# MohamedAbou-Taleb/Iterative-Linear-Quadratic-Regulator

Hardware: AMD Instinct MI355X
Metric: iLQR iterations/sec (batch=4096, T=200, n=4 m=1); backward-pass HBM GB/s (higher is better)
Workload: dtype f32; 1 GPU; c3: under-actuated double pendulum swing-up (run_iLQR_UA_MPC.py params), n=4 m=1 N=200 rk4, batch 4096 trajectories per GPU, 10 parallel line-search alphas per pass covering the 10 reference trials, fixed iterations; batch_per_gpu=4096, horizon=200, n_alpha=10, n_trials=10

## Files before the change

### iterative-linear-quadratic-regulator_amd/csrc/backward_fused16.hpp

```cpp
#pragma once

namespace ilqr {

template <typename T, int TPW, bool PK> struct FusedCfg;
template <> struct FusedCfg<float, 16, false> { static constexpr int P = 8, RU = 8; };
#ifndef ILQR_PK_RU
#define ILQR_PK_RU 5
#endif
#ifndef ILQR_PK_PAD
#define ILQR_PK_PAD 0
#endif
template <> struct FusedCfg<float, 16, true> { static constexpr int P = 4, RU = ILQR_PK_RU; };
template <> struct FusedCfg<double, 16, false> { static constexpr int P = 4, RU = 4; };
template <> struct FusedCfg<float, 4, false> { static constexpr int P = 3, RU = 4; };
template <> struct FusedCfg<double, 4, false> { static constexpr int P = 3, RU = 3; };

template <int NU> constexpr int fused_tl() { return NU == 2 ? 68 : 52; }
template <bool PK, int NU> constexpr int fused_unit_scalars() { return (PK ? 128 : 64) * fused_tl<NU>() + (PK ? 64 * ILQR_PK_PAD : 0); }
template <typename T, int TPW, bool PK, int NU> constexpr int fused_ru() { return (PK && NU == 2 && FusedCfg<T, TPW, PK>::RU > 4) ? 4 : FusedCfg<T, TPW, PK>::RU; }
template <typename T, int TPW, bool PK, int NU = 1> constexpr int fused_lds_bytes() {
    return fused_ru<T, TPW, PK, NU>() * fused_unit_scalars<PK, NU>() * (int)sizeof(T) + (fused_ru<T, TPW, PK, NU>() + 4 + 32 + 4) * 4;
}
static_assert(fused_lds_bytes<float, 16, true, 1>() <= 160 * 1024 && fused_lds_bytes<float, 16, true, 2>() <= 160 * 1024 &&
              fused_lds_bytes<float, 16, false, 2>() <= 160 * 1024 && fused_lds_bytes<double, 16, false, 2>() <= 160 * 1024, "LDS ring exceeds a CU");
template <typename T, int TPW, bool PK> constexpr int fused_threads() { return 64 * (TPW / 4 + FusedCfg<T, TPW, PK>::P); }

template <typename T, int NU> struct FusedStep;
template <> struct FusedStep<float, 1> {
    using Tile = TileQ;
    static ILQR_DEV void load(Tile& t, const float* tp, int i, int j, int l16) {
        const float4 s = *reinterpret_cast<const float4*>(tp + 4 * j);
        const float4 v = *reinterpret_cast<const float4*>(tp + 32 + 4 * j);
        t.skj[0] = s.x; t.skj[1] = s.y; t.skj[2] = s.z; t.skj[3] = s.w;
        t.vj[0] = v.x; t.vj[1] = v.y; t.vj[2] = v.z; t.vj[3] = v.w;
        t.a = tp[l16];
        t.lxx = tp[16 + l16];
        t.c = tp[32 + l16];
    }
    static ILQR_DEV void step(const Tile& c, const LaneConst<float>& lc, int i, int j, float& V, float& vx, float& out, bool& pd) {
        RawTileQ none;
        const i32x4 srd = {0, 0, 0, 0};
        const TileOffsets off = {0, 0, 0};
        float Kj, kff;
        tile16_step_f32<false>(c, lc, V, vx, Kj, kff, pd, none, srd, off, 0);
        out = (i == 0) ? Kj : kff;
    }
    static ILQR_DEV void step_box(const Tile& c, const LaneConst<float>& lc, int i, int j, float u, float lo, float hi,
                                  float& V, float& vx, float& out, bool& pd) {
        RawTileQ none;
        const i32x4 srd = {0, 0, 0, 0};
        const TileOffsets off = {0, 0, 0};
        float Kj, kff;
        tile16_step_f32<false, true>(c, lc, V, vx, Kj, kff, pd, none, srd, off, 0, u, lo, hi);
        out = (i == 0) ? Kj : kff;
    }
};
template <> struct FusedStep<double, 1> {
    using Tile = Tile16<double>;
    static ILQR_DEV void load(Tile& t, const double* tp, int i, int j, int l16) { tile16_load_lds(t, tp, i, j, l16); }
    static ILQR_DEV void step(const Tile& c, const LaneConst<double>& lc, int i, int j, double& V, double& vx, double& out, bool& pd) {
        double Kj, kff;
        tile16_step<double, false>(c, lc, 0.0, V, vx, Kj, kff, pd);
        out = (i == 0) ? Kj : kff;
    }
    static ILQR_DEV void step_box(const Tile& c, const LaneConst<double>& lc, int i, int j, double u, double lo, double hi,
                                  double& V, double& vx, double& out, bool& pd) {
        double Kj, kff;
        tile16_step<double, false, true>(c, lc, 0.0, V, vx, Kj, kff, pd, u, lo, hi);
        out = (i == 0) ? Kj : kff;
    }
};
template <> struct FusedStep<float, 2> {
    using Tile = TileQ2;
    static ILQR_DEV void load(Tile& t, const float* tp, int i, int j, int l16) { tileq2_load_lds(t, tp, i, j, l16); }
    static ILQR_DEV void step(const Tile& c, const LaneConst<float>& lc, int i, int j, float& V, float& vx, float& out, bool& pd) {
        const GainSel sel = GainSel::of(i, j);
        tile16m2_step_f32(c, lc, sel, V, vx, out, pd);
    }
};
template <typename T> struct FusedStep<T, 2> {
    using Tile = Tile16M2<T>;
    using V4 = typename Vec4<T>::type;
    static ILQR_DEV void load(Tile& t, const T* tp, int i, int j, int l16) {
        const V4 si = *reinterpret_cast<const V4*>(tp + 4 * i);
        const V4 sj = *reinterpret_cast<const V4*>(tp + 4 * j);
        const V4 g0 = *reinterpret_cast<const V4*>(tp + 32 + 8 * j);
        const V4 g1 = *reinterpret_cast<const V4*>(tp + 36 + 8 * j);
        t.ski[0] = si.x; t.ski[1] = si.y; t.ski[2] = si.z; t.ski[3] = si.w;
        t.skj[0] = sj.x; t.skj[1] = sj.y; t.skj[2] = sj.z; t.skj[3] = sj.w;
        t.gj[0] = g0.x; t.gj[1] = g0.y; t.gj[2] = g0.z; t.gj[3] = g0.w;
        t.gj[4] = g1.x; t.gj[5] = g1.y; t.gj[6] = g1.z; t.gj[7] = g1.w;
        const T* gi = tp + 32 + 8 * i;
        t.gi[0] = gi[0]; t.gi[1] = gi[1]; t.gi[3] = gi[3]; t.gi[4] = gi[4];
        t.lxx = tp[16 + l16];
    }
    static ILQR_DEV void step(const Tile& c, const LaneConst<T>& lc, int i, int j, T& V, T& vx, T& out, bool& pd) {
        T K0, K1, k0, k1;
        tile16m2_step<T, false>(c, lc.m0, lc.m1, T(0), V, vx, K0, K1, k0, k1, pd);
        out = (i == 0) ? K0 : ((i == 1) ? K1 : ((j == 0) ? k0 : k1));
    }
};

ILQR_DEV void compiler_fence() { asm volatile("" ::: "memory"); }
ILQR_DEV int lds_peek(const int* p) { return __hip_atomic_load(p, __ATOMIC_RELAXED, __HIP_MEMORY_SCOPE_WORKGROUP); }
ILQR_DEV void lds_poke(int* p, int v) { __hip_atomic_store(p, v, __ATOMIC_RELAXED, __HIP_MEMORY_SCOPE_WORKGROUP); }

template <typename T, typename Dyn, int INTEG, int TPW, bool PK, bool BOX, bool HET> struct FusedRoles {
    static constexpr int NX = Dyn::NX, NU = Dyn::NU;
    static_assert(!BOX || (NU == 1 && fused_tl<1>() > kTile16), "control limits: n_u = 1, u_t in the tile's padding");
    static_assert((NU == 1 && NX >= 2 && NX <= 4) || (NX == 4 && NU == 2), "the fused sweep serves the DPP tiles: n_u = 1, or (4, 2)");
    static_assert(TPW == 16 || TPW == 4, "16 or 4 trajectories per workgroup");
    static_assert(!PK || (sizeof(T) == 4 && TPW == 16 && INTEG != ILQR_INT_BACKWARD_EULER), "pair producers: fp32, 16-trajectory workgroups, explicit integrators");
    using Cfg = FusedCfg<T, TPW, PK>;
    static constexpr int P = Cfg::P, RU = fused_ru<T, TPW, PK, NU>(), TL = fused_tl<NU>();
    static constexpr int NV = (NU == 2 ? kTile16M2 : kTile16) / 4;
    static constexpr int NSW = TPW / 4;
    static constexpr int UT = PK ? 128 : 64;
    static constexpr int US = UT / TPW;
    static constexpr int UNIT = fused_unit_scalars<PK, NU>();
    static constexpr int PS = 2 * TL + ILQR_PK_PAD;
    static constexpr int R = gain_record(NX, NU);
    using PL = ParamLayout<Dyn::NSYS, NX, NU>;
    using V4 = typename Vec4<T>::type;
    static ILQR_DEV constexpr int tile_off(int r, int tl) { return PK ? ((r / 2) * TPW + tl) * PS + (r % 2) * TL : (r * TPW + tl) * TL; }
    static ILQR_DEV constexpr int step_off(int r) { return PK ? (r / 2) * TPW * PS + (r % 2) * TL : r * TPW * TL; }

    struct Lds {
        T* ring;
        int* ready;
        int* done;
        int* s_slot;
        int* s_stat;
    };
    static ILQR_DEV Lds carve(unsigned char* base) {
        Lds L;
        L.ring = reinterpret_cast<T*>(base);
        L.ready = reinterpret_cast<int*>(base + (size_t)RU * UNIT * sizeof(T));
        L.done = L.ready + RU;
        L.s_slot = L.done + 4;
        L.s_stat = L.s_slot + 16;
        return L;
    }

    static ILQR_DEV void head(const KArgs<T>& a, const Lds& L, int b0, int lane, bool do_select, bool count) {
        bool still = false;
        if (lane < 16) {
            const int b = b0 + lane;
            int slot = 0, st = -1;
            if (lane < TPW && b < a.B) {
                if (do_select) {
                    still = select_candidates(a, b, true, slot, st);
                } else {
                    st = a.status[b];
                    slot = a.cur_slot[b];
                }
                a.cur_slot[b] = traj_active(st) ? 0 : slot;
            }
            L.s_slot[lane] = slot;
            L.s_stat[lane] = st;
        } else if (lane < 16 + RU + 4) {
            L.ready[lane - 16] = 0;
        }
        if (do_select && count) {
            const unsigned long long m = __ballot(still);
            if (lane == 0 && m) atomicAdd(&a.counters[a.counter_idx], (int)__popcll(m));
            if (blockIdx.x == 0 && lane == 0) a.counters[(a.counter_idx + 1) % kCounterRing] = 0;
        }
    }
    static ILQR_DEV bool any_active(const Lds& L) {
        bool any = false;
#pragma unroll
        for (int q = 0; q < 16; ++q) any = any || traj_active(L.s_stat[q]);
        return any;
    }

    static ILQR_DEV void sweep(const KArgs<T>& a, const Lds& L, int b0, int wave, int lane, ClockProbe& cp) {
        const size_t B = a.B;
        const int N = a.N;
        const int tid = threadIdx.x;
        (void)tid;
        __builtin_amdgcn_s_setprio(2);
        const int l16 = lane & 15, i = l16 >> 2, j = l16 & 3;
        const int tl = 4 * wave + (lane >> 4);
        const int gidx = b0 + tl;
        const bool valid = gidx < a.B;
        const int b = valid ? gidx : a.B - 1;
        const int st = L.s_stat[tl];
        const bool act = valid && traj_active(st);
        const int slot = act ? L.s_slot[tl] : 0;
        T ph[HET ? PL::TOTAL : 1];
        if constexpr (HET) {
#pragma unroll
            for (int q = 0; q < PL::TOTAL; ++q) ph[q] = a.params[q];
            load_row<PL::Q>(ph, a.rows, B, b);
        }
        const T* __restrict__ pp = HET ? ph : a.params;
        T xN[NX];
        vec_load<T, NX>(a.X + vec_at(B, N + 1, NX, slot, N, b), xN);
        if (act && slot != 0 && l16 == 0) vec_store<T, NX>(a.X + vec_at(B, N + 1, NX, 0, N, b), xN);
        T V = T(0), vx = T(0);
        {
            T g[NX], H[NX][NX];
            Cost<T, Dyn>::l_f_x(pp, xN, g);
            Cost<T, Dyn>::l_f_xx(pp, xN, H);
#pragma unroll
            for (int ii = 0; ii < NX; ++ii) {
                if (j == ii) vx = g[ii];
#pragma unroll
                for (int jj = 0; jj < NX; ++jj)
                    if (i == ii && j == jj) V = H[ii][jj];
            }
        }
        const unsigned gain_bytes = (unsigned)((size_t)N * B * R * sizeof(T));
        const __amdgpu_buffer_rsrc_t rgain = make_rsrc(a.gains, gain_bytes);
        const int rstride = (int)(B * R * sizeof(T));
        constexpr bool DROP = sizeof(T) == 4 || ILQR_DROP_ALL;
        const bool storer = act && (NU == 1 ? ((i == 0 && j < NX) || l16 == 4) : (i < 2 || (i == 2 && j < 2)));
        const int rec_slot = NU == 1 ? (i == 0 ? j : NX) : (i < 2 ? 4 * i + j : 8 + j);
        const int rec_off = (storer || !DROP) ? (int)((b * R + rec_slot) * sizeof(T)) : 0x7ffffff0;
        LaneConst<T> lc;
        lc.m0 = T(j == 0);
        lc.m1 = T(j == 1);
        lc.tr_byte = 4 * ((lane & 48) | (j << 2) | i);
        bool all_pd = true;
        using FS = FusedStep<T, NU>;
        T blo = T(0), bhi = T(0);
        if constexpr (BOX) box_bounds<1>(a.lim, a.B, b, &blo, &bhi);
        typename FS::Tile tq[2];
        T uq[2] = {T(0), T(0)};
        auto load = [&](int q, const T* tp) {
            FS::load(tq[q], tp, i, j, l16);
            if constexpr (BOX) uq[q] = tp[kTile16];
        };
        int goff = (N - 1) * rstride;
        auto unit_base = [&](int k) -> const T* { return L.ring + (size_t)(k % RU) * UNIT + tile_off(0, tl); };
        constexpr auto step_off = [](int r) { return PK ? (r / 2) * TPW * PS + (r % 2) * TL : r * TPW * TL; };
        auto one_step = [&](int q) {
            T out;
            bool pd;
            if constexpr (BOX) FS::step_box(tq[q], lc, i, j, uq[q], blo, bhi, V, vx, out, pd);
            else FS::step(tq[q], lc, i, j, V, vx, out, pd);
            all_pd = all_pd && pd;
            if (DROP || storer) buf_store1(rgain, rec_off, uniform(goff), out);
            goff -= rstride;
        };
#ifdef ILQR_FUSED_STAMPS
        const long long st_t0 = __builtin_readcyclecounter();
        long long st_spin = 0;
#endif
        while (lds_peek(&L.ready[0]) < 1) __builtin_amdgcn_s_sleep(1);
        compiler_fence();
#ifdef ILQR_FUSED_STAMPS
        const long long st_first = __builtin_readcyclecounter();
#endif
        load(0, unit_base(0));
        const int n_full = N / US, rem = N % US;
        for (int k = 0; k < n_full; ++k) {
            const T* ub = unit_base(k);
            const bool more = (k + 1) * US < N;
            int flag = 0;
#pragma unroll
            for (int r = 0; r < US; ++r) {
                if (r == US - 2 && more) flag = lds_peek(&L.ready[(k + 1) % RU]);
                if (r < US - 1) {
                    load((r + 1) & 1, ub + step_off(r + 1));
                } else if (more) {
#ifdef ILQR_FUSED_STAMPS
                    const long long w0 = __builtin_readcyclecounter();
#endif
                    while (flag < k + 2) {
                        __builtin_amdgcn_s_sleep(1);
                        flag = lds_peek(&L.ready[(k + 1) % RU]);
                    }
                    compiler_fence();
#ifdef ILQR_FUSED_STAMPS
                    st_spin += __builtin_readcyclecounter() - w0;
#endif
                    load(0, unit_base(k + 1));
                }
                one_step(r & 1);
            }
            compiler_fence();
            if (lane == 0) lds_poke(&L.done[wave], k + 1);
        }
        if (rem) {
            const T* ub = unit_base(n_full);
#pragma unroll
            for (int r = 0; r < US - 1; ++r) {
                if (r < rem) {
                    if (r + 1 < rem) load((r + 1) & 1, ub + step_off(r + 1));
                    one_step(r & 1);
                }
            }
        }
#ifdef ILQR_FUSED_STAMPS
        if (a.probe && blockIdx.x == 7 && tid == 0) {
            a.probe[5] = st_first - st_t0;
            a.probe[6] = st_spin;
            a.probe[7] = __builtin_readcyclecounter() - st_first;
        }
#endif
        cp.stop(a.probe, 0);
        if (act && l16 == 0 && !all_pd) a.status[b] = st | ILQR_TRAJ_FLAG_NON_PD;
    }

    static ILQR_DEV void produce(const KArgs<T>& a_, const Lds& L, int b0, int pw, int lane) {
        struct { int B; T dt; T* X; T* U; const T* params; const T* rows; } a = {a_.B, a_.dt, a_.X, a_.U, a_.params, a_.rows};
        const size_t B = a.B;
        const int N = a_.N;
        const int n_units = (N + US - 1) / US;
        if constexpr (PK) {
        using T2 = pair_f32;
        using Dyn2 = typename Dyn::template rebind<T2>;
        const int tl = lane % TPW, r2 = lane / TPW;
        const int gidx = b0 + tl;
        const bool valid = gidx < a.B;
        const int b = valid ? gidx : a.B - 1;
        const bool actb = valid && traj_active(L.s_stat[tl]);
        const int slot = actb ? L.s_slot[tl] : 0;
        const bool move = actb && slot != 0;
        T pl[PL::TOTAL];
#pragma unroll
        for (int q = 0; q < PL::TOTAL; ++q) pl[q] = a.params[q];
        if constexpr (HET) load_row<PL::Q>(pl, a.rows, B, b);
        const SplatParams p{pl};
        const T2 dt2 = a.dt;
        for (int k = pw; k < n_units; k += P) {
            const int ta = N - 1 - k * US - 2 * r2, tb = ta - 1;
            const bool ina = ta >= 0, inb = tb >= 0;
            const int tta = ina ? ta : 0, ttb = inb ? tb : 0;
            T xa[NX], ua[NU], xb[NX], ub[NU];
            vec_load<T, NX>(a.X + vec_at(B, N + 1, NX, slot, tta, b), xa);
            vec_load<T, NU>(a.U + vec_at(B, N, NU, slot, tta, b), ua);
            vec_load<T, NX>(a.X + vec_at(B, N + 1, NX, slot, ttb, b), xb);
            vec_load<T, NU>(a.U + vec_at(B, N, NU, slot, ttb, b), ub);
            if (move && ina) {
                vec_store<T, NX>(a.X + vec_at(B, N + 1, NX, 0, tta, b), xa);
                vec_store<T, NU>(a.U + vec_at(B, N, NU, 0, tta, b), ua);
            }
            if (move && inb) {
                vec_store<T, NX>(a.X + vec_at(B, N + 1, NX, 0, ttb, b), xb);
                vec_store<T, NU>(a.U + vec_at(B, N, NU, 0, ttb, b), ub);
            }
            T2 x[NX], u[NU], xn[NX], fx[NX][NX], fu[NX][NU];
#pragma unroll
            for (int q = 0; q < NX; ++q) { x[q].x = xa[q]; x[q].y = xb[q]; }
#pragma unroll
            for (int q = 0; q < NU; ++q) { u[q].x = ua[q]; u[q].y = ub[q]; }
            Stepper<T2, Dyn2>::step_jac(INTEG, p, dt2, x, u, xn, fx, fu);
            T2 gxn[NX], gu1[NU], lxxn[NX][NX], luxn[NU][NX], luu[NU][NU];
            Cost<T2, Dyn2>::grad(p, dt2, x, u, gxn, gu1);
            Cost<T2, Dyn2>::hess(p, dt2, x, u, lxxn, luxn, luu);
            V4 tile_a[NV], tile_b[NV];
            tile16_fill<T, NX, NU>([](T2 v) { return v.x; }, fx, fu, gxn, gu1, lxxn, luxn, luu, tile_a);
            tile16_fill<T, NX, NU>([](T2 v) { return v.y; }, fx, fu, gxn, gu1, lxxn, luxn, luu, tile_b);
            if (k >= RU) {
                const int need = k - RU + 1;
                auto slowest = [&]() {
                    int m = lds_peek(&L.done[0]);
#pragma unroll
                    for (int q = 1; q < NSW; ++q) m = min(m, lds_peek(&L.done[q]));
                    return m;
                };
                while (slowest() < need) __builtin_amdgcn_s_sleep(2);
            }
            compiler_fence();
            V4* dst = reinterpret_cast<V4*>(L.ring + (size_t)(k % RU) * UNIT + tile_off(2 * r2, tl));
            if (ina) {
#pragma unroll
                for (int q = 0; q < NV; ++q) dst[q] = tile_a[q];
            }
            if (inb) {
#pragma unroll
                for (int q = 0; q < NV; ++q) dst[TL / 4 + q] = tile_b[q];
            }
            if constexpr (BOX) {
                T* dt_ = reinterpret_cast<T*>(dst);
                if (ina) dt_[kTile16] = ua[0];
                if (inb) dt_[TL + kTile16] = ub[0];
            }
            compiler_fence();
            if (lane == 0) lds_poke(&L.ready[k % RU], k + 1);
        }
        } else {
        const int tl = lane % TPW, r = lane / TPW;
        const int gidx = b0 + tl;
        const bool valid = gidx < a.B;
        const int b = valid ? gidx : a.B - 1;
        const bool actb = valid && traj_active(L.s_stat[tl]);
        const int slot = actb ? L.s_slot[tl] : 0;
        const bool move = actb && slot != 0;
        T p[PL::TOTAL];
#pragma unroll
        for (int q = 0; q < PL::TOTAL; ++q) p[q] = a.params[q];
        if constexpr (HET) load_row<PL::Q>(p, a.rows, B, b);
        for (int k = pw; k < n_units; k += P) {
            const int t = N - 1 - k * US - r;
            const bool inr = t >= 0;
            const int tt = inr ? t : 0;
            T x[NX], u[NU];
            vec_load<T, NX>(a.X + vec_at(B, N + 1, NX, slot, tt, b), x);
            vec_load<T, NU>(a.U + vec_at(B, N, NU, slot, tt, b), u);
            if (move && inr) {
                vec_store<T, NX>(a.X + vec_at(B, N + 1, NX, 0, tt, b), x);
                vec_store<T, NU>(a.U + vec_at(B, N, NU, 0, tt, b), u);
            }
            T xn[NX], fx[NX][NX], fu[NX][NU];
            Stepper<T, Dyn>::step_jac(INTEG, p, a.dt, x, u, xn, fx, fu);
            V4 tile[NV];
            tile16_pack<T, Dyn>(p, a.dt, x, u, fx, fu, tile);
            if (k >= RU) {
                const int need = k - RU + 1;
                auto slowest = [&]() {
                    int m = lds_peek(&L.done[0]);
#pragma unroll
                    for (int q = 1; q < NSW; ++q) m = min(m, lds_peek(&L.done[q]));
                    return m;
                };
                while (slowest() < need) __builtin_amdgcn_s_sleep(2);
            }
            compiler_fence();
            if (inr) {
                constexpr int NQ = NV * (int)sizeof(V4) / 16;
                vec_u4 w[NQ];
                __builtin_memcpy(w, tile, sizeof(V4) * NV);
                vec_u4* dst = reinterpret_cast<vec_u4*>(L.ring + (size_t)(k % RU) * UNIT + tile_off(r, tl));
#pragma unroll
                for (int q = 0; q < NQ; ++q) dst[q] = w[q];
                if constexpr (BOX) reinterpret_cast<T*>(dst)[kTile16] = u[0];
            }
            compiler_fence();
            if (lane == 0) lds_poke(&L.ready[k % RU], k + 1);
        }
        }
    }
};

template <typename T, typename Dyn, int INTEG, int TPW, bool PK, bool BOX = false>
struct FusedWG : FusedRoles<T, Dyn, INTEG, TPW, PK, BOX, false> {};
template <typename T, typename Dyn, int INTEG, int TPW, bool PK, bool BOX = false>
struct FusedWGHet : FusedRoles<T, Dyn, INTEG, TPW, PK, BOX, true> {};

template <typename T, typename Dyn, int INTEG, int TPW, bool PK, bool BOX = false, bool HET = false>
__global__ void __launch_bounds__((fused_threads<T, TPW, PK>())) backward_fused16_kernel(KArgs<T> a) {
    using W = std::conditional_t<HET, FusedWGHet<T, Dyn, INTEG, TPW, PK, BOX>, FusedWG<T, Dyn, INTEG, TPW, PK, BOX>>;
    extern __shared__ __attribute__((aligned(16))) unsigned char fused_lds[];
    const typename W::Lds L = W::carve(fused_lds);
    const int tid = threadIdx.x, wave = tid >> 6, lane = tid & 63;
    const int b0 = blockIdx.x * TPW;
    ClockProbe cp;
    cp.start();
    if (wave == 0) W::head(a, L, b0, lane, a.fuse_select != 0, true);
    __syncthreads();
    if (!W::any_active(L)) return;
    if (wave < W::NSW) W::sweep(a, L, b0, wave, lane, cp);
    else W::produce(a, L, b0, wave - W::NSW, lane);
}

}
```

### iterative-linear-quadratic-regulator_amd/csrc/kernels.hpp

```cpp
#pragma once
#include "dynamics.hpp"

namespace ilqr {

#ifndef ILQR_NT_TILE_STORE
#define ILQR_NT_TILE_STORE 0
#endif
#ifndef ILQR_NT_TILE_LOAD
#define ILQR_NT_TILE_LOAD 0
#endif
#ifndef ILQR_DROP_ALL
#define ILQR_DROP_ALL 0
#endif
constexpr int kMaxAlpha = 16;
constexpr int kCounterRing = 64;
constexpr int kBoxMaxU = 2;
constexpr int kALMaxX = 4;

template <typename T> struct Limits {
    T u_lo[kBoxMaxU], u_hi[kBoxMaxU];
    T x_lo[kALMaxX], x_hi[kALMaxX];
    int al_mask;
    const T* u_lo_rows;
    const T* u_hi_rows;
// ... 35 lines not shown
#pragma unroll
    for (int j = 0; j < NU; ++j) {
        lo[j] = rl ? rl[(size_t)j * B + b] : a.u_lo[j];
        hi[j] = rl ? rh[(size_t)j * B + b] : a.u_hi[j];
    }
}

template <int NH, typename T> ILQR_DEV void load_row(T* p, const T* __restrict__ rows, size_t B, int b) {
#pragma unroll
    for (int q = 0; q < NH; ++q) p[q] = rows[(size_t)q * B + b];
}

constexpr int gain_record(int nx, int nu) { return ((nu * nx + nu) + 3) / 4 * 4; }

ILQR_DEV bool traj_active(int status) { return (status & 0xff) == ILQR_TRAJ_ACTIVE; }

template <typename T> ILQR_DEV T clamp_keep_nan(T v, T lo, T hi) { return v < lo ? lo : (v > hi ? hi : v); }

ILQR_DEV size_t vec_at(size_t B, int Tn, int C, int slot, int t, size_t b) {
    return ((((size_t)slot * Tn + t) * B) + b) * C;
}
typedef unsigned int vec_u4 __attribute__((ext_vector_type(4)));
typedef unsigned int vec_u2 __attribute__((ext_vector_type(2)));
constexpr int vec_piece(int bytes) { return bytes % 16 == 0 ? 16 : bytes % 8 == 0 ? 8 : 4; }
constexpr int vec_pieces(int bytes) { return bytes / vec_piece(bytes); }
template <typename T, int C> ILQR_DEV void vec_load(const T* __restrict__ p, T* o) {
    constexpr int BYTES = C * (int)sizeof(T), PB = vec_piece(BYTES), NP = BYTES / PB;
    if constexpr (PB == 16) {
        vec_u4 v[NP];
#pragma unroll
        for (int k = 0; k < NP; ++k) v[k] = reinterpret_cast<const vec_u4*>(p)[k];
        __builtin_memcpy(o, v, BYTES);
    } else if constexpr (PB == 8) {
        vec_u2 v[NP];
#pragma unroll
        for (int k = 0; k < NP; ++k) v[k] = reinterpret_cast<const vec_u2*>(p)[k];
        __builtin_memcpy(o, v, BYTES);
    } else {
#pragma unroll
        for (int i = 0; i < C; ++i) o[i] = p[i];
    }
}
template <typename T, int C> ILQR_DEV void vec_store(T* __restrict__ p, const T* v) {
    constexpr int BYTES = C * (int)sizeof(T), PB = vec_piece(BYTES), NP = BYTES / PB;
    if constexpr (PB == 16) {
        vec_u4 w[NP];
        __builtin_memcpy(w, v, BYTES);
#pragma unroll
        for (int k = 0; k < NP; ++k) reinterpret_cast<vec_u4*>(p)[k] = w[k];
    } else if constexpr (PB == 8) {
        vec_u2 w[NP];
        __builtin_memcpy(w, v, BYTES);
#pragma unroll
        for (int k = 0; k < NP; ++k) reinterpret_cast<vec_u2*>(p)[k] = w[k];
    } else {
#pragma unroll
        for (int i = 0; i < C; ++i) p[i] = v[i];
    }
}

struct ClockProbe {
    long long c0, r0;
    ILQR_DEV void start() { c0 = __builtin_readcyclecounter(); r0 = wall_clock64(); }
    ILQR_DEV void stop(long long* probe, int slot) const {
        if (probe && threadIdx.x == 0) {
            const long long c1 = __builtin_readcyclecounter(), r1 = wall_clock64();
            const size_t wg = (size_t)blockIdx.y * gridDim.x + blockIdx.x;
            if (wg == 0) { probe[2 * slot] = c1 - c0; probe[2 * slot + 1] = r1 - r0; }
            if (wg < 65536) {
                long long* q = probe + 8 + ((size_t)slot * 65536 + wg) * 4;
                q[0] = r0; q[1] = r1; q[2] = c1 - c0;
                q[3] = (long long)__builtin_amdgcn_s_getreg((4 ) | (0 << 6) | (31 << 11)) |
                       ((long long)__builtin_amdgcn_s_getreg((20 ) | (0 << 6) | (3 << 11)) << 32);
            }
        }
    }
};

}
#include "backward_tile16.hpp"
#include "backward_tile16m2.hpp"
namespace ilqr {

template <typename TS, int NX, int NU, typename T, typename Pick>
ILQR_DEV void tile16_fill(Pick pick, const T (*fx)[NX], const T (*fu)[NU], const T* gxn, const T* gu1, const T (*lxxn)[NX],
                          const T (*luxn)[NX], const T (*luu)[NU], typename Vec4<TS>::type* tile) {
    static_assert((NX >= 2 && NX <= 4 && NU == 1) || (NX == 4 && NU == 2), "tile packing: n_x <= 4 with n_u = 1, or (4, 2)");
    auto F = [&](int i, int j) -> TS { return (i < NX && j < NX) ? pick(fx[i < NX ? i : 0][j < NX ? j : 0]) : TS(0); };
    auto L = [&](int i, int j) -> TS { return (i < NX && j < NX) ? pick(lxxn[i < NX ? i : 0][j < NX ? j : 0]) : TS(0); };
#pragma unroll
    for (int c = 0; c < 4; ++c) {
        tile[c].x = F((c + 0) & 3, c); tile[c].y = F((c + 1) & 3, c);
        tile[c].z = F((c + 2) & 3, c); tile[c].w = F((c + 3) & 3, c);
    }
#pragma unroll
    for (int i = 0; i < 4; ++i) {
        tile[4 + i].x = L(i, 0); tile[4 + i].y = L(i, 1);
        tile[4 + i].z = L(i, 2); tile[4 + i].w = L(i, 3);
    }
    if constexpr (NU == 1) {
#pragma unroll
        for (int j = 0; j < 4; ++j) {
            const int jj = j < NX ? j : 0;
            tile[8 + j].x = j < NX ? pick(fu[jj][0]) : TS(0);
            tile[8 + j].y = j < NX ? pick(gxn[jj]) : TS(0);
            tile[8 + j].z = j < NX ? pick(luxn[0][jj]) : TS(0);
            tile[8 + j].w = (j == 0) ? pick(gu1[0]) : ((j == 1) ? pick(luu[0][0]) : TS(0));
        }
    } else {
#pragma unroll
        for (int j = 0; j < 4; ++j) {
            tile[8 + 2 * j].x = pick(fu[j][0]); tile[8 + 2 * j].y = pick(fu[j][NU - 1]);
            tile[8 + 2 * j].z = pick(gxn[j]); tile[8 + 2 * j].w = pick(luxn[0][j]);
            tile[9 + 2 * j].x = pick(luxn[NU - 1][j]);
            tile[9 + 2 * j].y = (j == 0) ? pick(gu1[0]) : ((j == 1) ? TS(0.5) * (pick(luu[0][NU - 1]) + pick(luu[NU - 1][0])) : TS(0));
            tile[9 + 2 * j].z = (j == 0) ? pick(gu1[NU - 1]) : ((j == 1) ? pick(luu[NU - 1][NU - 1]) : TS(0));
            tile[9 + 2 * j].w = (j == 0) ? pick(luu[0][0]) : TS(0);
        }
    }
}

template <typename T, typename Dyn, typename P>
ILQR_DEV void tile16_pack(P p, T dt, const T* x, const T* u, const T (*fx)[Dyn::NX],
                          const T (*fu)[Dyn::NU], typename Vec4<T>::type* tile) {
    constexpr int NX = Dyn::NX, NU = Dyn::NU;
    T gxn[NX], gu1[NU], lxxn[NX][NX], luxn[NU][NX], luu[NU][NU];
    Cost<T, Dyn>::grad(p, dt, x, u, gxn, gu1);
    Cost<T, Dyn>::hess(p, dt, x, u, lxxn, luxn, luu);
    tile16_fill<T, NX, NU>([](T v) { return v; }, fx, fu, gxn, gu1, lxxn, luxn, luu, tile);
}

template <typename T, int NX> struct ALBounds {
    T lo[NX], hi[NX];
    int mask;
    ILQR_DEV ALBounds(const Limits<T>& a, size_t B, int b) : mask(a.al_mask) {
        const T* __restrict__ rl = a.x_lo_rows;
        const T* __restrict__ rh = a.x_hi_rows;
#pragma unroll
        for (int i = 0; i < NX; ++i) {
            lo[i] = rl ? rl[(size_t)i * B + b] : a.x_lo[i];
            hi[i] = rl ? rh[(size_t)i * B + b] : a.x_hi[i];
        }
    }
};
template <typename T, int NX> ILQR_DEV T al_constraint(const ALBounds<T, NX>& a, const T* x, int q) {
    return q < NX ? x[q < NX ? q : 0] - a.hi[q < NX ? q : 0] : a.lo[q < NX ? 0 : q - NX] - x[q < NX ? 0 : q - NX];
}
template <typename T> ILQR_DEV T al_pos(T v) { return v > T(0) ? v : T(0); }
template <typename T, int NX> ILQR_DEV void al_load_lam(const KArgs<T>& a, size_t B, int b, int t, T* lam) {
#pragma unroll
    for (int q = 0; q < 2 * NX; ++q) lam[q] = ((a.lim.al_mask >> q) & 1) ? a.lam[((size_t)t * 2 * NX + q) * B + b] : T(0);
}
template <typename T, int NX> ILQR_DEV T al_phi(const ALBounds<T, NX>& a, const T* x, const T* lam, T rho) {
    T s = T(0);
#pragma unroll
    for (int q = 0; q < 2 * NX; ++q) {
        if ((a.mask >> q) & 1) {
            const T m = al_pos(lam[q] + rho * al_constraint<T, NX>(a, x, q));
            s += (m * m - lam[q] * lam[q]) / (T(2) * rho);
        }
    }
    return s;
}
template <typename T, int NX>
ILQR_DEV void al_expand(const ALBounds<T, NX>& a, const T* x, const T* lam, T rho, T* g, T (*H)[NX]) {
#pragma unroll
    for (int q = 0; q < 2 * NX; ++q) {
        if ((a.mask >> q) & 1) {
            const int j = q % NX;
            const T v = lam[q] + rho * al_constraint<T, NX>(a, x, q);
            const T m = al_pos(v);
            if (q < NX) g[j] += m;
            else g[j] -= m;
            if (v > T(0)) H[j][j] += rho;
        }
    }
}

template <int E, typename T> ILQR_DEV void load_expansion(const T* src, size_t B, T* tile) {
#pragma unroll
    for (int e = 0; e < E; ++e) tile[e] = src[(size_t)e * B];
}
template <typename T, int NX> ILQR_DEV void load_terminal(const T* term, size_t B, int b, T* Vx, T (*Vxx)[NX]) {
#pragma unroll
    for (int i = 0; i < NX; ++i) Vx[i] = term[(size_t)i * B + b];
#pragma unroll
    for (int i = 0; i < NX; ++i)
#pragma unroll
        for (int j = 0; j < NX; ++j) Vxx[i][j] = term[(size_t)(NX + i * NX + j) * B + b];
}
template <typename T, int NX, int NU> ILQR_DEV void store_gains(T* rec, const T (*K)[NX], const T* k) {
#pragma unroll
    for (int i = 0; i < NU; ++i)
#pragma unroll
        for (int j = 0; j < NX; ++j) rec[i * NX + j] = K[i][j];
#pragma unroll
    for (int i = 0; i < NU; ++i) rec[NU * NX + i] = k[i];
}

template <typename T, typename Dyn, bool TILE16, int INTEG, bool HET = false>
__global__ void __launch_bounds__(TILE16 ? 64 : 256) linearize_kernel(KArgs<T> a) {
    constexpr int NX = Dyn::NX, NU = Dyn::NU;
    constexpr int E = 2 * NX * NX + 2 * NX * NU + NX + NU + NU * NU;
    using PL = ParamLayout<Dyn::NSYS, NX, NU>;
    const size_t idx = (size_t)blockIdx.x * blockDim.x + threadIdx.x;
    const size_t B = a.B;
    const int t = (int)(idx / B);
    const int b = (int)(idx % B);
    const bool inr = t <= a.N;
    const int st_raw = inr ? a.status[b] : 0;
    const int slot_raw = inr ? a.cur_slot[b] : 0;
    const bool live = inr && traj_active(st_raw);
// ... 1306 lines not shown
```

### iterative-linear-quadratic-regulator_amd/csrc/ops.hpp

```cpp
#pragma once
#include <hip/hip_runtime.h>
#include <hip/hip_ext.h>

#include <algorithm>
#include <cstdlib>

#include "kernels_wave.hpp"
#include "backward_mfma16.hpp"
#include "forward_mfma16.hpp"
#include "policy_rollout.hpp"
#include "sample_controls.hpp"

namespace ilqr {

constexpr size_t kDescriptorMax = 0x7ffffff0ull;

struct LaunchEvents { hipEvent_t a = nullptr, b = nullptr; };
inline LaunchEvents& launch_events() { static thread_local LaunchEvents e; return e; }
#define ILQR_LAUNCH(kern, grid, block, lds, stream, ...)                                                     \
    do {                                                                                                     \
        LaunchEvents& le_ = launch_events();                                                                 \
        hipExtLaunchKernelGGL(kern, grid, block, lds, stream, le_.a, le_.b, 0, __VA_ARGS__);                 \
        le_ = LaunchEvents();                                                                                \
    } while (0)
// ... 10 lines not shown
    } while (0)

template <auto K> bool allow_dynamic_lds(int bytes) {
    static const bool ok = [bytes] {
        const bool r = hipFuncSetAttribute((const void*)K, hipFuncAttributeMaxDynamicSharedMemorySize, bytes) == hipSuccess;
        (void)hipGetLastError();
        return r;
    }();
    return ok;
}

inline bool forward_plain() {
    static const bool v = getenv("ILQR_FORWARD_PLAIN") != nullptr;
    return v;
}
template <typename T> bool ring_rollout_ok(const KArgs<T>& a, int nx, int nu) {
    const size_t bytes_x = (size_t)a.n_slots * (a.N + 1) * nx * a.B * sizeof(T);
    const size_t bytes_g = (size_t)a.N * a.B * gain_record(nx, nu) * sizeof(T);
    return !forward_plain() && std::max(bytes_x, bytes_g) <= kDescriptorMax;
}

template <typename T> struct Ops {
    void (*linearize[5])(const KArgs<T>&, hipStream_t) = {};
    void (*backward)(const KArgs<T>&, hipStream_t) = nullptr;
    void (*forward[5])(const KArgs<T>&, hipStream_t) = {};
    void (*fused[5])(const KArgs<T>&, hipStream_t) = {};
    void (*persist[5])(const KArgs<T>&, const PArgs<T>&, hipStream_t) = {};
    bool persist_any_batch[5] = {};
    bool persist_big = false;
    void (*eval)(const EvalArgs<T>&, hipStream_t) = nullptr;
    void (*mpc_advance)(const MpcArgs<T>&, hipStream_t) = nullptr;
    int n_dev_params = 0;
    int n_sys_dev = 0;
    int lin_stride = 0;
    bool tile16 = false;
    int tile_scalars = 0;
    bool lin_aos = false;
    bool canonical = false;
    bool const_lin = false;
    bool (*sweep_reads_sparse)(T mu) = nullptr;
    void (*linearize_box[5])(const KArgs<T>&, hipStream_t) = {};
    void (*backward_box)(const KArgs<T>&, hipStream_t) = nullptr;
    void (*forward_box[5])(const KArgs<T>&, hipStream_t) = {};
    bool fused_box = false;
    bool het = false;
    bool persist_het[5] = {};
    void (*linearize_al[5])(const KArgs<T>&, hipStream_t) = {};
    void (*forward_al[5])(const KArgs<T>&, hipStream_t) = {};
    void (*al_update)(const KArgs<T>&, const ALArgs<T>&, hipStream_t) = nullptr;
    void (*al_cost)(const KArgs<T>&, const ALArgs<T>&, hipStream_t) = nullptr;
    void (*mpc_advance_al)(const MpcALArgs<T>&, hipStream_t) = nullptr;
    void (*policy)(const PolicyArgs<T>&, hipStream_t) = nullptr;
    void (*policy_noise)(const PolicyArgs<T>&, const NoiseArgs<T>&, hipStream_t) = nullptr;
    void (*sample_begin)(const SampleArgs<T>&, hipStream_t) = nullptr;
    void (*sample_rollout)(const SampleArgs<T>&, const NoiseArgs<T>&, hipStream_t) = nullptr;
    void (*sample_update)(const SampleArgs<T>&, hipStream_t) = nullptr;
};

template <typename T, int NX, int NU, typename = void> struct has_fwd_in { static constexpr bool value = false; };
template <typename T, int NX, int NU> struct has_fwd_in<T, NX, NU, decltype((void)sizeof(FwdIn<T, NX, NU>))> {
    static constexpr bool value = true;
};

#ifndef ILQR_RING_INTEG_MASK
#define ILQR_RING_INTEG_MASK 0x1f
#endif
#ifndef ILQR_FUSE_INTEG_MASK
#define ILQR_FUSE_INTEG_MASK 0x1f
#endif
inline int persist_small_max();
#ifndef ILQR_PERSIST_INTEG_MASK
#define ILQR_PERSIST_INTEG_MASK 0x1f
#endif
#ifndef ILQR_NO_PAIR_PRODUCERS
#define ILQR_NO_PAIR_PRODUCERS 0
#endif
template <typename Dyn, typename = void> struct has_rebind { static constexpr bool value = false; };
template <typename Dyn> struct has_rebind<Dyn, std::void_t<typename Dyn::template rebind<float>>> { static constexpr bool value = true; };

template <typename T, typename Dyn, int I, bool BX, bool HT> void launch_fused_kernel(const KArgs<T>& a, hipStream_t s) {
    constexpr bool CAN_PK = sizeof(T) == 4 && I != ILQR_INT_BACKWARD_EULER && has_rebind<Dyn>::value && !ILQR_NO_PAIR_PRODUCERS;
    constexpr auto K16 = backward_fused16_kernel<T, Dyn, I, 16, false, BX, HT>;
    constexpr auto K4 = backward_fused16_kernel<T, Dyn, I, 4, false, BX, HT>;
    constexpr int LDS16 = fused_lds_bytes<T, 16, false, Dyn::NU>(), LDS4 = fused_lds_bytes<T, 4, false, Dyn::NU>();
    bool ok = allow_dynamic_lds<K16>(LDS16) && allow_dynamic_lds<K4>(LDS4);
    if constexpr (CAN_PK)
        ok = ok && allow_dynamic_lds<backward_fused16_kernel<T, Dyn, I, 16, true, BX, HT>>(fused_lds_bytes<T, 16, true, Dyn::NU>());
    (void)ok;
    static const int force = getenv("ILQR_FUSED_TPW") ? atoi(getenv("ILQR_FUSED_TPW")) : 0;
    static const bool no_pk = getenv("ILQR_FUSED_PAIRS") != nullptr && atoi(getenv("ILQR_FUSED_PAIRS")) == 0;
    const bool small = force ? force == 4 : a.B <= persist_small_max();
    if (small) {
        ILQR_LAUNCH(K4, dim3((a.B + 3) / 4), dim3(fused_threads<T, 4, false>()), LDS4, s, a);
        return;
    }
    if constexpr (CAN_PK) {
        if (!no_pk) {
            ILQR_LAUNCH((backward_fused16_kernel<T, Dyn, I, 16, true, BX, HT>), dim3((a.B + 15) / 16), dim3(fused_threads<T, 16, true>()),
                        (fused_lds_bytes<T, 16, true, Dyn::NU>()), s, a);
            return;
        }
    }
    ILQR_LAUNCH(K16, dim3((a.B + 15) / 16), dim3(fused_threads<T, 16, false>()), LDS16, s, a);
}

template <typename T, typename Dyn, int I, bool BX, bool HT>
void launch_persist_kernel(const KArgs<T>& a, const PArgs<T>& pa, hipStream_t s) {
    constexpr bool BIG = I != ILQR_INT_BACKWARD_EULER && has_rebind<Dyn>::value && !ILQR_NO_PAIR_PRODUCERS;
    constexpr auto K4 = ilqr_persistent_kernel<T, Dyn, I, 4, false, BX, HT>;
    constexpr int LDS4 = fused_lds_bytes<T, 4, false, Dyn::NU>();
    bool ok = allow_dynamic_lds<K4>(LDS4);
    if constexpr (BIG)
        ok = ok && allow_dynamic_lds<ilqr_persistent_kernel<T, Dyn, I, 16, true, BX, HT>>(fused_lds_bytes<T, 16, true, Dyn::NU>());
    (void)ok;
    if constexpr (BIG) {
        if (a.B > persist_small_max()) {
            ILQR_LAUNCH((ilqr_persistent_kernel<T, Dyn, I, 16, true, BX, HT>), dim3((a.B + 15) / 16), dim3(fused_threads<T, 16, true>()),
                        (fused_lds_bytes<T, 16, true, Dyn::NU>()), s, a, pa);
            return;
        }
    }
    ILQR_LAUNCH(K4, dim3((a.B + 3) / 4), dim3(fused_threads<T, 4, false>()), LDS4, s, a, pa);
}

template <typename Dyn> constexpr bool box_system() {
    return Dyn::ID == ILQR_SYS_PENDULUM || Dyn::ID == ILQR_SYS_UA_DOUBLE_PENDULUM || Dyn::ID == ILQR_SYS_DOUBLE_PENDULUM;
}
#ifndef ILQR_PERSIST_HET_INTEG_MASK
#define ILQR_PERSIST_HET_INTEG_MASK 0x1f
#endif

template <typename T, typename Dyn, bool TILE, int I, bool HETS, bool AL = false>
void launch_linearize(const KArgs<T>& a, hipStream_t s) {
    static_assert(!(AL && TILE), "the state-limited expansion has the generic layout only");
    const size_t total = (size_t)a.B * (a.N + 1);
    constexpr int TPB = TILE ? 64 : 256;
    const dim3 grid((unsigned)((total + TPB - 1) / TPB)), block(TPB);
    if constexpr (AL)
        ILQR_LAUNCH_HET(HETS, a.het, (linearize_al_kernel<T, Dyn, I>), (linearize_al_kernel<T, Dyn, I, true>), grid, block, 0, s, a);
    else
        ILQR_LAUNCH_HET(HETS, a.het, (linearize_kernel<T, Dyn, TILE, I>), (linearize_kernel<T, Dyn, TILE, I, true>), grid, block, 0, s, a);
}

template <typename T, typename Dyn, int I, bool RING, bool BOX, bool AL, bool HETS>
void launch_forward(const KArgs<T>& a, hipStream_t s) {
    const dim3 grid((a.B + 63) / 64, a.n_pass), block(64);
    if constexpr (RING && !AL) {
        if (ring_rollout_ok(a, Dyn::NX, Dyn::NU)) {
            if constexpr (BOX)
                ILQR_LAUNCH_HET(HETS, a.het, (forward_ring_kernel_box<T, Dyn, I>), (forward_ring_kernel_box_het<T, Dyn, I>), grid, block, 0, s, a);
            else
                ILQR_LAUNCH_HET(HETS, a.het, (forward_ring_kernel<T, Dyn, I>), (forward_ring_kernel_het<T, Dyn, I>), grid, block, 0, s, a);
            return;
        }
    }
    if constexpr (AL)
        ILQR_LAUNCH_HET(HETS, a.het, (forward_kernel_al<T, Dyn, I>), (forward_kernel_al_het<T, Dyn, I>), grid, block, 0, s, a);
    else if constexpr (BOX)
        ILQR_LAUNCH_HET(HETS, a.het, (forward_kernel_box<T, Dyn, I>), (forward_kernel_box_het<T, Dyn, I>), grid, block, 0, s, a);
    else
        ILQR_LAUNCH_HET(HETS, a.het, (forward_kernel<T, Dyn, I>), (forward_kernel_het<T, Dyn, I>), grid, block, 0, s, a);
}

template <typename T, typename Dyn> void launch_policy(const PolicyArgs<T>& a, hipStream_t s) {
    const dim3 grid((a.S + 63) / 64, a.B), block(64);
    if (a.srows) ILQR_LAUNCH((policy_rollout_kernel<T, Dyn, true>), grid, block, 0, s, a);
    else ILQR_LAUNCH((policy_rollout_kernel<T, Dyn, false>), grid, block, 0, s, a);
}
template <typename T, typename Dyn> void launch_policy_noise(const PolicyArgs<T>& a, const NoiseArgs<T>& nz, hipStream_t s) {
    const dim3 grid((a.S + 63) / 64, a.B), block(64);
    if (a.srows) ILQR_LAUNCH((policy_noise_kernel<T, Dyn, true>), grid, block, 0, s, a, nz);
    else ILQR_LAUNCH((policy_noise_kernel<T, Dyn, false>), grid, block, 0, s, a, nz);
}

template <typename T, typename Dyn> void launch_sample_begin(const SampleArgs<T>& a, hipStream_t s) {
    const size_t n = (size_t)a.B * a.N * Dyn::NU;
    ILQR_LAUNCH((sample_nominal_kernel<T>), dim3((unsigned)((n + 255) / 256)), dim3(256), 0, s, a.Ub, a.U, a.cur_slot, a.B, a.N, Dyn::NU);
}
template <typename T, typename Dyn> void launch_sample_rollout(const SampleArgs<T>& a, const NoiseArgs<T>& nz, hipStream_t s) {
    ILQR_LAUNCH((sample_rollout_kernel<T, Dyn>), dim3((a.S + 63) / 64, a.B), dim3(64), 0, s, a, nz);
}
template <typename T, typename Dyn> void launch_sample_update(const SampleArgs<T>& a, hipStream_t s) {
    const int rows = a.N * Dyn::NU;
    const LaunchEvents le = launch_events();
    launch_events() = LaunchEvents{le.a, nullptr};
    ILQR_LAUNCH((sample_weights_kernel<T>), dim3(a.B), dim3(64), 0, s, a);
    launch_events() = LaunchEvents{nullptr, le.b};
    if (a.mode == ILQR_SAMPLE_SOFTMIN) ILQR_LAUNCH((sample_softmin_kernel<T, Dyn::NU>), dim3(a.N, a.B), dim3(64), 0, s, a);
    else ILQR_LAUNCH((sample_best_kernel<T>), dim3((rows + 63) / 64, a.B), dim3(64), 0, s, a, (int)Dyn::NU);
}

template <typename T, typename Dyn, bool TILE, int INTEG> void set_integrator_ops(Ops<T>& o) {
    constexpr bool SMALL = all_integrators<Dyn>::value;
    constexpr bool FUSED_BOX = box_system<Dyn>() && Dyn::NU == 1;
    if constexpr (TILE && FUSED_BOX) o.fused_box = true;
    constexpr bool HETS = box_system<Dyn>();
    if constexpr (HETS) o.het = true;
    constexpr int I = (SMALL || INTEG == ILQR_INT_DISCRETE) ? INTEG : ILQR_INT_EULER;
    constexpr bool RING = has_fwd_in<T, Dyn::NX, Dyn::NU>::value && ((ILQR_RING_INTEG_MASK >> I) & 1);
    o.linearize[INTEG] = launch_linearize<T, Dyn, TILE, I, HETS>;
    if constexpr (TILE && ((ILQR_FUSE_INTEG_MASK >> I) & 1)) {
// ... 177 lines not shown
```

Baseline: 29.82 million iLQR iterations/sec.

## Drop constant l_xx from LDS ring tiles and deepen the ring

For fp32 single-control systems with the default quadratic cost, the state Hessian l_xx is constant (Q*dt). It is no longer packed into each ring tile; consumers compute it once per lane from the parameters. This shrinks each tile from 52 to 36 scalars, which cuts LDS write and read traffic per step and cuts producer packing work. The freed LDS is spent on more ring slots (12/8/6) so a workgroup's LDS footprint does not fall and occupancy placement stays at one workgroup per CU. The catch is that it only holds for cost models whose l_xx does not depend on state, which the code gates on has_custom_cost.

```diff
diff --git a/iterative-linear-quadratic-regulator_amd/csrc/backward_fused16.hpp b/iterative-linear-quadratic-regulator_amd/csrc/backward_fused16.hpp
--- a/iterative-linear-quadratic-regulator_amd/csrc/backward_fused16.hpp
+++ b/iterative-linear-quadratic-regulator_amd/csrc/backward_fused16.hpp
@@ -2,27 +2,51 @@
 
 namespace ilqr {
 
+#ifndef ILQR_SC_RUC
+#define ILQR_SC_RUC 12
+#endif
+#ifndef ILQR_PK_RUC
+#define ILQR_PK_RUC 8
+#endif
+#ifndef ILQR_T4_RUC
+#define ILQR_T4_RUC 6
+#endif
 template <typename T, int TPW, bool PK> struct FusedCfg;
-template <> struct FusedCfg<float, 16, false> { static constexpr int P = 8, RU = 8; };
+template <> struct FusedCfg<float, 16, false> { static constexpr int P = 8, RU = 8, RUC = ILQR_SC_RUC; };
 #ifndef ILQR_PK_RU
 #define ILQR_PK_RU 5
 #endif
 #ifndef ILQR_PK_PAD
 #define ILQR_PK_PAD 0
 #endif
-template <> struct FusedCfg<float, 16, true> { static constexpr int P = 4, RU = ILQR_PK_RU; };
-template <> struct FusedCfg<double, 16, false> { static constexpr int P = 4, RU = 4; };
-template <> struct FusedCfg<float, 4, false> { static constexpr int P = 3, RU = 4; };
-template <> struct FusedCfg<double, 4, false> { static constexpr int P = 3, RU = 3; };
-
-template <int NU> constexpr int fused_tl() { return NU == 2 ? 68 : 52; }
-template <bool PK, int NU> constexpr int fused_unit_scalars() { return (PK ? 128 : 64) * fused_tl<NU>() + (PK ? 64 * ILQR_PK_PAD : 0); }
-template <typename T, int TPW, bool PK, int NU> constexpr int fused_ru() { return (PK && NU == 2 && FusedCfg<T, TPW, PK>::RU > 4) ? 4 : FusedCfg<T, TPW, PK>::RU; }
-template <typename T, int TPW, bool PK, int NU = 1> constexpr int fused_lds_bytes() {
-    return fused_ru<T, TPW, PK, NU>() * fused_unit_scalars<PK, NU>() * (int)sizeof(T) + (fused_ru<T, TPW, PK, NU>() + 4 + 32 + 4) * 4;
+template <> struct FusedCfg<float, 16, true> { static constexpr int P = 4, RU = ILQR_PK_RU, RUC = ILQR_PK_RUC; };
+template <> struct FusedCfg<double, 16, false> { static constexpr int P = 4, RU = 4, RUC = 4; };
+template <> struct FusedCfg<float, 4, false> { static constexpr int P = 3, RU = 4, RUC = ILQR_T4_RUC; };
+template <> struct FusedCfg<double, 4, false> { static constexpr int P = 3, RU = 3, RUC = 3; };
+
+template <typename T, typename Dyn> constexpr bool fused_const_lxx() { return sizeof(T) == 4 && Dyn::NU == 1 && !has_custom_cost<Dyn>::value; }
+template <int NU, bool CL = false> constexpr int fused_tl() { return NU == 2 ? 68 : (CL ? 36 : 52); }
+template <bool PK, int NU, bool CL = false> constexpr int fused_unit_scalars() { return (PK ? 128 : 64) * fused_tl<NU, CL>() + (PK ? 64 * ILQR_PK_PAD : 0); }
+template <typename T, int TPW, bool PK, int NU, bool CL = false> constexpr int fused_ru() {
+    return CL ? FusedCfg<T, TPW, PK>::RUC : ((PK && NU == 2 && FusedCfg<T, TPW, PK>::RU > 4) ? 4 : FusedCfg<T, TPW, PK>::RU);
+}
+template <typename T, int TPW, bool PK, int NU = 1, bool CL = false> constexpr int fused_lds_bytes() {
+    return fused_ru<T, TPW, PK, NU, CL>() * fused_unit_scalars<PK, NU, CL>() * (int)sizeof(T) + (fused_ru<T, TPW, PK, NU, CL>() + 4 + 32 + 4) * 4;
+}
+template <typename T, typename Dyn, int TPW, bool PK> constexpr int fused_lds_for() {
+    return fused_lds_bytes<T, TPW, PK, Dyn::NU, fused_const_lxx<T, Dyn>()>();
 }
 static_assert(fused_lds_bytes<float, 16, true, 1>() <= 160 * 1024 && fused_lds_bytes<float, 16, true, 2>() <= 160 * 1024 &&
-              fused_lds_bytes<float, 16, false, 2>() <= 160 * 1024 && fused_lds_bytes<double, 16, false, 2>() <= 160 * 1024, "LDS ring exceeds a CU");
+              fused_lds_bytes<float, 16, false, 2>() <= 160 * 1024 && fused_lds_bytes<double, 16, false, 2>() <= 160 * 1024 &&
+              fused_lds_bytes<float, 16, true, 1, true>() <= 160 * 1024 && fused_lds_bytes<float, 16, false, 1, true>() <= 160 * 1024 &&
+              fused_lds_bytes<float, 4, false, 1, true>() <= 160 * 1024, "LDS ring exceeds a CU");
+#ifndef ILQR_DEPTH_LADDER
+static_assert(fused_lds_bytes<float, 16, true, 1, true>() >= fused_lds_bytes<float, 16, true, 1>() &&
+              fused_lds_bytes<float, 16, false, 1, true>() >= fused_lds_bytes<float, 16, false, 1>() &&
+              fused_lds_bytes<float, 4, false, 1, true>() >= fused_lds_bytes<float, 4, false, 1>(),
+              "the compact tile must not lower a workgroup's LDS: the one-workgroup-per-CU placement rests on it");
+#endif
+static_assert(ILQR_SC_RUC + 20 <= 64 && ILQR_PK_RUC + 20 <= 64 && ILQR_T4_RUC + 20 <= 64, "ring slots: the head clears their flags with one wave");
 template <typename T, int TPW, bool PK> constexpr int fused_threads() { return 64 * (TPW / 4 + FusedCfg<T, TPW, PK>::P); }
 
 template <typename T, int NU> struct FusedStep;
@@ -36,6 +60,15 @@
         t.a = tp[l16];
         t.lxx = tp[16 + l16];
         t.c = tp[32 + l16];
+    }
+    static ILQR_DEV void load_compact(Tile& t, const float* tp, int i, int j, int l16, float lxx) {
+        const float4 s = *reinterpret_cast<const float4*>(tp + 4 * j);
+        const float4 v = *reinterpret_cast<const float4*>(tp + 16 + 4 * j);
+        t.skj[0] = s.x; t.skj[1] = s.y; t.skj[2] = s.z; t.skj[3] = s.w;
+        t.vj[0] = v.x; t.vj[1] = v.y; t.vj[2] = v.z; t.vj[3] = v.w;
+        t.a = tp[l16];
+        t.lxx = lxx;
+        t.c = tp[16 + l16];
     }
     static ILQR_DEV void step(const Tile& c, const LaneConst<float>& lc, int i, int j, float& V, float& vx, float& out, bool& pd) {
         RawTileQ none;
@@ -107,17 +140,19 @@
 
 template <typename T, typename Dyn, int INTEG, int TPW, bool PK, bool BOX, bool HET> struct FusedRoles {
     static constexpr int NX = Dyn::NX, NU = Dyn::NU;
-    static_assert(!BOX || (NU == 1 && fused_tl<1>() > kTile16), "control limits: n_u = 1, u_t in the tile's padding");
+    static constexpr bool CL = fused_const_lxx<T, Dyn>();
+    static constexpr int TS = NU == 2 ? kTile16M2 : (CL ? 32 : kTile16);
+    static_assert(!BOX || (NU == 1 && fused_tl<1, CL>() > TS), "control limits: n_u = 1, u_t in the tile's padding");
     static_assert((NU == 1 && NX >= 2 && NX <= 4) || (NX == 4 && NU == 2), "the fused sweep serves the DPP tiles: n_u = 1, or (4, 2)");
     static_assert(TPW == 16 || TPW == 4, "16 or 4 trajectories per workgroup");
     static_assert(!PK || (sizeof(T) == 4 && TPW == 16 && INTEG != ILQR_INT_BACKWARD_EULER), "pair producers: fp32, 16-trajectory workgroups, explicit integrators");
     using Cfg = FusedCfg<T, TPW, PK>;
-    static constexpr int P = Cfg::P, RU = fused_ru<T, TPW, PK, NU>(), TL = fused_tl<NU>();
-    static constexpr int NV = (NU == 2 ? kTile16M2 : kTile16) / 4;
+    static constexpr int P = Cfg::P, RU = fused_ru<T, TPW, PK, NU, CL>(), TL = fused_tl<NU, CL>();
+    static constexpr int NV = TS / 4;
     static constexpr int NSW = TPW / 4;
     static constexpr int UT = PK ? 128 : 64;
     static constexpr int US = UT / TPW;
-    static constexpr int UNIT = fused_unit_scalars<PK, NU>();
+    static constexpr int UNIT = fused_unit_scalars<PK, NU, CL>();
     static constexpr int PS = 2 * TL + ILQR_PK_PAD;
     static constexpr int R = gain_record(NX, NU);
     using PL = ParamLayout<Dyn::NSYS, NX, NU>;
@@ -224,13 +259,20 @@
         lc.tr_byte = 4 * ((lane & 48) | (j << 2) | i);
         bool all_pd = true;
         using FS = FusedStep<T, NU>;
+        T lxxc = T(0);
+        if constexpr (CL) {
+            const bool in = i < NX && j < NX;
+            const T qs = a.params[PL::QS + (in ? i * NX + j : 0)];
+            lxxc = in ? qs * a.dt : T(0);
+        }
         T blo = T(0), bhi = T(0);
         if constexpr (BOX) box_bounds<1>(a.lim, a.B, b, &blo, &bhi);
         typename FS::Tile tq[2];
         T uq[2] = {T(0), T(0)};
         auto load = [&](int q, const T* tp) {
-            FS::load(tq[q], tp, i, j, l16);
-            if constexpr (BOX) uq[q] = tp[kTile16];
+            if constexpr (CL) FS::load_compact(tq[q], tp, i, j, l16, lxxc);
+            else FS::load(tq[q], tp, i, j, l16);
+            if constexpr (BOX) uq[q] = tp[TS];
         };
         int goff = (N - 1) * rstride;
         auto unit_base = [&](int k) -> const T* { return L.ring + (size_t)(k % RU) * UNIT + tile_off(0, tl); };
@@ -352,8 +394,8 @@
             Cost<T2, Dyn2>::grad(p, dt2, x, u, gxn, gu1);
             Cost<T2, Dyn2>::hess(p, dt2, x, u, lxxn, luxn, luu);
             V4 tile_a[NV], tile_b[NV];
-            tile16_fill<T, NX, NU>([](T2 v) { return v.x; }, fx, fu, gxn, gu1, lxxn, luxn, luu, tile_a);
-            tile16_fill<T, NX, NU>([](T2 v) { return v.y; }, fx, fu, gxn, gu1, lxxn, luxn, luu, tile_b);
+            tile16_fill<T, NX, NU, !CL>([](T2 v) { return v.x; }, fx, fu, gxn, gu1, lxxn, luxn, luu, tile_a);
+            tile16_fill<T, NX, NU, !CL>([](T2 v) { return v.y; }, fx, fu, gxn, gu1, lxxn, luxn, luu, tile_b);
             if (k >= RU) {
                 const int need = k - RU + 1;
                 auto slowest = [&]() {
@@ -376,8 +418,8 @@
             }
             if constexpr (BOX) {
                 T* dt_ = reinterpret_cast<T*>(dst);
-                if (ina) dt_[kTile16] = ua[0];
-                if (inb) dt_[TL + kTile16] = ub[0];
+                if (ina) dt_[TS] = ua[0];
+                if (inb) dt_[TL + TS] = ub[0];
             }
             compiler_fence();
             if (lane == 0) lds_poke(&L.ready[k % RU], k + 1);
@@ -408,7 +450,7 @@
             T xn[NX], fx[NX][NX], fu[NX][NU];
             Stepper<T, Dyn>::step_jac(INTEG, p, a.dt, x, u, xn, fx, fu);
             V4 tile[NV];
-            tile16_pack<T, Dyn>(p, a.dt, x, u, fx, fu, tile);
+            tile16_pack<T, Dyn, !CL>(p, a.dt, x, u, fx, fu, tile);
             if (k >= RU) {
                 const int need = k - RU + 1;
                 auto slowest = [&]() {
@@ -427,7 +469,7 @@
                 vec_u4* dst = reinterpret_cast<vec_u4*>(L.ring + (size_t)(k % RU) * UNIT + tile_off(r, tl));
 #pragma unroll
                 for (int q = 0; q < NQ; ++q) dst[q] = w[q];
-                if constexpr (BOX) reinterpret_cast<T*>(dst)[kTile16] = u[0];
+                if constexpr (BOX) reinterpret_cast<T*>(dst)[TS] = u[0];
             }
             compiler_fence();
             if (lane == 0) lds_poke(&L.ready[k % RU], k + 1);
diff --git a/iterative-linear-quadratic-regulator_amd/csrc/kernels.hpp b/iterative-linear-quadratic-regulator_amd/csrc/kernels.hpp
--- a/iterative-linear-quadratic-regulator_amd/csrc/kernels.hpp
+++ b/iterative-linear-quadratic-regulator_amd/csrc/kernels.hpp
@@ -141,10 +141,12 @@
 #include "backward_tile16m2.hpp"
 namespace ilqr {
 
-template <typename TS, int NX, int NU, typename T, typename Pick>
+template <typename TS, int NX, int NU, bool LXX = true, typename T, typename Pick>
 ILQR_DEV void tile16_fill(Pick pick, const T (*fx)[NX], const T (*fu)[NU], const T* gxn, const T* gu1, const T (*lxxn)[NX],
                           const T (*luxn)[NX], const T (*luu)[NU], typename Vec4<TS>::type* tile) {
     static_assert((NX >= 2 && NX <= 4 && NU == 1) || (NX == 4 && NU == 2), "tile packing: n_x <= 4 with n_u = 1, or (4, 2)");
+    static_assert(LXX || NU == 1, "the compact tile: n_u = 1");
+    constexpr int M = LXX ? 8 : 4;
     auto F = [&](int i, int j) -> TS { return (i < NX && j < NX) ? pick(fx[i < NX ? i : 0][j < NX ? j : 0]) : TS(0); };
     auto L = [&](int i, int j) -> TS { return (i < NX && j < NX) ? pick(lxxn[i < NX ? i : 0][j < NX ? j : 0]) : TS(0); };
 #pragma unroll
@@ -152,19 +154,22 @@
         tile[c].x = F((c + 0) & 3, c); tile[c].y = F((c + 1) & 3, c);
         tile[c].z = F((c + 2) & 3, c); tile[c].w = F((c + 3) & 3, c);
     }
-#pragma unroll
-    for (int i = 0; i < 4; ++i) {
-        tile[4 + i].x = L(i, 0); tile[4 + i].y = L(i, 1);
-        tile[4 + i].z = L(i, 2); tile[4 + i].w = L(i, 3);
+    (void)L;
+    if constexpr (LXX) {
+#pragma unroll
+        for (int i = 0; i < 4; ++i) {
+            tile[4 + i].x = L(i, 0); tile[4 + i].y = L(i, 1);
+            tile[4 + i].z = L(i, 2); tile[4 + i].w = L(i, 3);
+        }
     }
     if constexpr (NU == 1) {
 #pragma unroll
         for (int j = 0; j < 4; ++j) {
             const int jj = j < NX ? j : 0;
-            tile[8 + j].x = j < NX ? pick(fu[jj][0]) : TS(0);
-            tile[8 + j].y = j < NX ? pick(gxn[jj]) : TS(0);
-            tile[8 + j].z = j < NX ? pick(luxn[0][jj]) : TS(0);
-            tile[8 + j].w = (j == 0) ? pick(gu1[0]) : ((j == 1) ? pick(luu[0][0]) : TS(0));
+            tile[M + j].x = j < NX ? pick(fu[jj][0]) : TS(0);
+            tile[M + j].y = j < NX ? pick(gxn[jj]) : TS(0);
+            tile[M + j].z = j < NX ? pick(luxn[0][jj]) : TS(0);
+            tile[M + j].w = (j == 0) ? pick(gu1[0]) : ((j == 1) ? pick(luu[0][0]) : TS(0));
         }
     } else {
 #pragma unroll
@@ -179,14 +184,14 @@
     }
 }
 
-template <typename T, typename Dyn, typename P>
+template <typename T, typename Dyn, bool LXX = true, typename P>
 ILQR_DEV void tile16_pack(P p, T dt, const T* x, const T* u, const T (*fx)[Dyn::NX],
                           const T (*fu)[Dyn::NU], typename Vec4<T>::type* tile) {
     constexpr int NX = Dyn::NX, NU = Dyn::NU;
     T gxn[NX], gu1[NU], lxxn[NX][NX], luxn[NU][NX], luu[NU][NU];
     Cost<T, Dyn>::grad(p, dt, x, u, gxn, gu1);
     Cost<T, Dyn>::hess(p, dt, x, u, lxxn, luxn, luu);
-    tile16_fill<T, NX, NU>([](T v) { return v; }, fx, fu, gxn, gu1, lxxn, luxn, luu, tile);
+    tile16_fill<T, NX, NU, LXX>([](T v) { return v; }, fx, fu, gxn, gu1, lxxn, luxn, luu, tile);
 }
 
 template <typename T, int NX> struct ALBounds {
diff --git a/iterative-linear-quadratic-regulator_amd/csrc/ops.hpp b/iterative-linear-quadratic-regulator_amd/csrc/ops.hpp
--- a/iterative-linear-quadratic-regulator_amd/csrc/ops.hpp
+++ b/iterative-linear-quadratic-regulator_amd/csrc/ops.hpp
@@ -116,10 +116,10 @@
     constexpr bool CAN_PK = sizeof(T) == 4 && I != ILQR_INT_BACKWARD_EULER && has_rebind<Dyn>::value && !ILQR_NO_PAIR_PRODUCERS;
     constexpr auto K16 = backward_fused16_kernel<T, Dyn, I, 16, false, BX, HT>;
     constexpr auto K4 = backward_fused16_kernel<T, Dyn, I, 4, false, BX, HT>;
-    constexpr int LDS16 = fused_lds_bytes<T, 16, false, Dyn::NU>(), LDS4 = fused_lds_bytes<T, 4, false, Dyn::NU>();
+    constexpr int LDS16 = fused_lds_for<T, Dyn, 16, false>(), LDS4 = fused_lds_for<T, Dyn, 4, false>();
     bool ok = allow_dynamic_lds<K16>(LDS16) && allow_dynamic_lds<K4>(LDS4);
     if constexpr (CAN_PK)
-        ok = ok && allow_dynamic_lds<backward_fused16_kernel<T, Dyn, I, 16, true, BX, HT>>(fused_lds_bytes<T, 16, true, Dyn::NU>());
+        ok = ok && allow_dynamic_lds<backward_fused16_kernel<T, Dyn, I, 16, true, BX, HT>>(fused_lds_for<T, Dyn, 16, true>());
     (void)ok;
     static const int force = getenv("ILQR_FUSED_TPW") ? atoi(getenv("ILQR_FUSED_TPW")) : 0;
     static const bool no_pk = getenv("ILQR_FUSED_PAIRS") != nullptr && atoi(getenv("ILQR_FUSED_PAIRS")) == 0;
@@ -131,7 +131,7 @@
     if constexpr (CAN_PK) {
         if (!no_pk) {
             ILQR_LAUNCH((backward_fused16_kernel<T, Dyn, I, 16, true, BX, HT>), dim3((a.B + 15) / 16), dim3(fused_threads<T, 16, true>()),
-                        (fused_lds_bytes<T, 16, true, Dyn::NU>()), s, a);
+                        (fused_lds_for<T, Dyn, 16, true>()), s, a);
             return;
         }
     }
@@ -142,15 +142,15 @@
 void launch_persist_kernel(const KArgs<T>& a, const PArgs<T>& pa, hipStream_t s) {
     constexpr bool BIG = I != ILQR_INT_BACKWARD_EULER && has_rebind<Dyn>::value && !ILQR_NO_PAIR_PRODUCERS;
     constexpr auto K4 = ilqr_persistent_kernel<T, Dyn, I, 4, false, BX, HT>;
-    constexpr int LDS4 = fused_lds_bytes<T, 4, false, Dyn::NU>();
+    constexpr int LDS4 = fused_lds_for<T, Dyn, 4, false>();
     bool ok = allow_dynamic_lds<K4>(LDS4);
     if constexpr (BIG)
-        ok = ok && allow_dynamic_lds<ilqr_persistent_kernel<T, Dyn, I, 16, true, BX, HT>>(fused_lds_bytes<T, 16, true, Dyn::NU>());
+        ok = ok && allow_dynamic_lds<ilqr_persistent_kernel<T, Dyn, I, 16, true, BX, HT>>(fused_lds_for<T, Dyn, 16, true>());
     (void)ok;
     if constexpr (BIG) {
         if (a.B > persist_small_max()) {
             ILQR_LAUNCH((ilqr_persistent_kernel<T, Dyn, I, 16, true, BX, HT>), dim3((a.B + 15) / 16), dim3(fused_threads<T, 16, true>()),
-                        (fused_lds_bytes<T, 16, true, Dyn::NU>()), s, a, pa);
+                        (fused_lds_for<T, Dyn, 16, true>()), s, a, pa);
             return;
         }
     }
```

Measured after the change: 29.43 million iLQR iterations/sec. -1.3%, worse.
